# ruanyyyyyyy/point-cloud-process

Hardware: AMD Instinct MI355X
Metric: correspondence-pairs/sec + ms/ICP-iter, 120k-pt KITTI pair (higher is better)
Workload: dtype f64; 1 GPU; point-to-point ICP iteration, 120000 x 120000 KITTI-shaped synthetic scan pair per GPU (BASELINE configs[1]); exact 1-NN via grid; nn=grid, pairs_per_gpu=1, points_src=120000, points_tgt=120000

## Files before the change

point-cloud-process_amd/csrc/pcr_grid_search.hip:

```cpp
#include <atomic>
#include <chrono>
#include <cmath>
#include <cstdlib>
#include <cstring>
#include "pcr_grid_dev.h"
#include "pcr_icp_step.h"

#ifndef PCR_HARD_SCAN_T
#define PCR_HARD_SCAN_T 192
#endif
constexpr unsigned int HARD_SCAN_T = PCR_HARD_SCAN_T;
constexpr int HARD_STACK = 160;
constexpr long long ID_NONE = 0x7fffffffffffffffll;
constexpr int H_NLIST = 32;
constexpr int H_CSTRIDE = 32;
__host__ __device__ static inline unsigned int hard_list_cap(long long nq) {
    const long long tiles = (nq + 15) / 16;
    return (unsigned int)(((tiles + H_NLIST - 1) / H_NLIST) * 16 + 64);
}

template <int G>
__device__ static inline void group_best(double& bd2, long long& bid, unsigned int& bpos) {
#pragma unroll
    for (int off = G / 2; off > 0; off >>= 1) {
// ... 136 lines not shown
    unsigned long long dbg_pairs;
    unsigned int dbg_passes;
    unsigned long long probe;
};

struct wt_pre {
    pcr_pt p;
    unsigned int seed_pos;
    wt_xyz seed_b;
};
__device__ __forceinline__ static void wtile_preload(const unsigned int tile, const int lane, const pcr_pt* __restrict__ q, const long long nq,
                                                     const unsigned int* __restrict__ res_pos, const wt_xyz* __restrict__ prev_xyz, wt_pre& P) {
    const long long qi = (long long)tile * WT_Q + (lane & (WT_Q - 1));
    P.seed_pos = POS_NONE;
    P.seed_b = wt_xyz{0.0, 0.0, 0.0};
    P.p.x = P.p.y = P.p.z = 0.0; P.p.id = 0;
    if (qi < nq) {
        if (prev_xyz) {
            P.seed_pos = res_pos[qi];
            P.seed_b = prev_xyz[qi];
        }
        P.p = q[qi];
    }
}

#ifndef PCR_WT_WAVES
#define PCR_WT_WAVES 4
#endif
__device__ __forceinline__ static void wtile_search(const pcr_grid_view& gv, wtile_lds* L, const unsigned int tile, const int lane, const wt_pre& P,
                                                    pcr_pt* __restrict__ q, const long long nq, const pcr_xform& x, const int has_x, const int write_back,
                                                    const double max_d2, const int gated, const unsigned int pcap, unsigned int* __restrict__ res_pos,
                                                    double* __restrict__ res_d2, unsigned long long* __restrict__ dbg,
                                                    const wt_xyz* __restrict__ prev_xyz, wt_state& S, const unsigned long long* probe_p = nullptr,
                                                    const unsigned int probe_stride = 0, const unsigned int probe_groups = 0, const unsigned int probe_total = 0) {
#if !PCR_WT_MFMA
    typedef float f2 __attribute__((ext_vector_type(2)));
#endif
    typedef float f4 __attribute__((ext_vector_type(4)));
    const pcr_pt* __restrict__ g_pts = as_global(gv.pts);
#ifdef PCR_WT_DIAG
    const unsigned long long t_start = dbg ? __builtin_amdgcn_s_memtime() : 0;
    unsigned long long t_ph[8] = {0, 0, 0, 0, 0, 0, 0, 0}, t_last = t_start;
#define WT_STAMP(i) do { if (dbg) { const unsigned long long t_now = __builtin_amdgcn_s_memtime(); t_ph[i] += t_now - t_last; t_last = t_now; } } while (0)
#define WT_WHY(v) do { why = (v); } while (0)
    int why = 0;
#else
#define WT_STAMP(i) do {} while (0)
#define WT_WHY(v) do {} while (0)
#endif
    const long long qi = (long long)tile * WT_Q + (lane & (WT_Q - 1));
    const bool qvalid = qi < nq;
    double ax = 0, ay = 0, az = 0;
    bool clamped = false;
    const unsigned int seed_pos = P.seed_pos;
    const wt_xyz seed_b = P.seed_b;
    if (qvalid) {
        const pcr_pt p = P.p;
        ax = p.x; ay = p.y; az = p.z;
        if (has_x) {
            xform_apply(x, p, &ax, &ay, &az);
            if (write_back && lane < WT_Q) {
                pcr_pt o;
                o.x = ax; o.y = ay; o.z = az; o.id = p.id;
                q[qi] = o;
            }
        }
        cell_coord(ax, gv.lo[0], gv.inv_cell0, &clamped);
        cell_coord(ay, gv.lo[1], gv.inv_cell0, &clamped);
        cell_coord(az, gv.lo[2], gv.inv_cell0, &clamped);
    }
    
    WT_STAMP(0);
    bool open = qvalid;
    const float gate2 = gated ? (float)max_d2 * (1.0f + 1e-6f) : INFINITY;
    float bound2 = gate2;
    unsigned int cand_pos = POS_NONE, won = POS_NONE;
    if (prev_xyz && qvalid && !clamped) {
        const unsigned int pp = seed_pos;
        if (pp != POS_NONE) {
            const wt_xyz b = seed_b;
            const double dx = ax - b.x, dy = ay - b.y, dz = az - b.z;
            const float up = (float)((dx * dx + dy * dy) + dz * dz) * (1.0f + 2e-7f) + 1e-37f;
            if (up < bound2) { bound2 = up; cand_pos = pp; }
        }
    }
    unsigned long long dbg_pairs = 0, probe_v = 0;
    unsigned int dbg_passes = 0, staged = 0;
    const int max_passes = prev_xyz ? WT_PASSES_SEEDED : WT_PASSES;
    unsigned int staged_done = 0;
    float ring = 1.0f;
#pragma unroll 1
    for (int pass = 0; pass < max_passes; ++pass) {
        const bool part = open && !clamped;
        if (!__any(part)) break;
        if (pass > 0 && staged_done > (unsigned int)WT_HEAVY_STOP) break;
        int mn[3], mx[3];
        {
            const float rho = (cand_pos != POS_NONE) ? sqrtf(bound2) * (1.0f + 1e-6f) : fminf((float)gv.cell0 * ring, sqrtf(gate2));
            const double rc = fmin((double)rho * gv.inv_cell0, 262144.0);
            const double tx = (ax - gv.lo[0]) * gv.inv_cell0, ty = (ay - gv.lo[1]) * gv.inv_cell0, tz = (az - gv.lo[2]) * gv.inv_cell0;
            const int cmax = (int)PCR_COORD_MAX;
            mn[0] = part ? max(0, min(cmax, (int)floor(tx - rc) + (int)PCR_COORD_BIAS)) : 0x7fffffff;
            mx[0] = part ? max(0, min(cmax, (int)floor(tx + rc) + (int)PCR_COORD_BIAS)) : -1;
            mn[1] = part ? max(0, min(cmax, (int)floor(ty - rc) + (int)PCR_COORD_BIAS)) : 0x7fffffff;
            mx[1] = part ? max(0, min(cmax, (int)floor(ty + rc) + (int)PCR_COORD_BIAS)) : -1;
            mn[2] = part ? max(0, min(cmax, (int)floor(tz - rc) + (int)PCR_COORD_BIAS)) : 0x7fffffff;
            mx[2] = part ? max(0, min(cmax, (int)floor(tz + rc) + (int)PCR_COORD_BIAS)) : -1;
        }
#pragma unroll
        for (int k = 0; k < 3; ++k) {
            int lo_k = row16_min(mn[k]), hi_k = row16_max(mx[k]);
            if (WT_Q >= 32) {
                lo_k = min(__builtin_amdgcn_readlane(lo_k, 0), __builtin_amdgcn_readlane(lo_k, 16));
                hi_k = max(__builtin_amdgcn_readlane(hi_k, 0), __builtin_amdgcn_readlane(hi_k, 16));
            }
            if (WT_Q == 64) {
                const int lo2 = min(__builtin_amdgcn_readlane(row16_min(mn[k]), 32), __builtin_amdgcn_readlane(row16_min(mn[k]), 48));
// ... 286 lines not shown
#pragma unroll
        for (int off = WT_Q; off < 64; off <<= 1) {
            const float om = __shfl_xor(fm, off, 64), os = __shfl_xor(fs, off, 64);
            const unsigned int op = __shfl_xor(bpos, off, 64);
            fs = fminf(fmaxf(fm, om), fminf(fs, os));
            if (om < fm) { fm = om; bpos = op; }
        }
        if (part) {
            float U = INFINITY;
            bool ambiguous = false;
            if (bpos != POS_NONE) {
                const float R = 0.5f * cellLf * (float)max(d0, max(d1, d2));
                const float e = 8.0f * 5.9604644775390625e-08f * R * (1.0f + 1e-6f);
                const float dhi = sqrtf(fm) * (1.0f + 2e-6f) + e;
                U = (dhi + e) * (dhi + e) * (1.0f + 2e-6f);
                ambiguous = fs <= U;
            }
            float db = fminf(fminf(0.5f * d0 * cellLf - fabsf(qxf), 0.5f * d1 * cellLf - fabsf(qyf)), 0.5f * d2 * cellLf - fabsf(qzf));
            db = fmaxf(db - cellLf * (float)max(d0, max(d1, d2)) * 4e-6f, 0.0f);
            const float reach2 = fminf(U, bound2);
            if (!ambiguous && reach2 <= db * db * (1.0f - 2e-6f)) {
                open = false;
                won = bpos;
                if (lane < WT_Q) {
                    if (res_d2) {
                        double dd = DBL_MAX;
                        if (bpos != POS_NONE) {
                            const pcr_pt bb = g_pts[bpos];
                            dd = dist2(ax, ay, az, bb);
                        }
                        res_d2[qi] = dd;
                    }
                    if (!prev_xyz || bpos != seed_pos) res_pos[qi] = bpos;
                }
            } else {
                WT_WHY(ambiguous ? 3 : 4);
                if (bpos != POS_NONE && U < bound2) {
                    bound2 = U;
                    cand_pos = bpos;
                }
            }
        }
        ring = ring == 0.0f ? 1.0f : ring * 4.0f;
    }
    WT_STAMP(6);
    S.ax = ax; S.ay = ay; S.az = az;
    S.qi = qi;
    S.bound2 = bound2;
    S.cand_pos = cand_pos;
    S.won = won;
    S.open = open; S.clamped = clamped; S.qvalid = qvalid;
    S.staged = staged;
    S.dbg_pairs = dbg_pairs; S.dbg_passes = dbg_passes;
    {
        const bool ok = lane < (int)probe_groups && (unsigned int)probe_v == probe_total / (probe_groups ? probe_groups : 1u) + ((unsigned int)lane < probe_total % (probe_groups ? probe_groups : 1u) ? 1u : 0u);
        S.probe = (probe_groups && __ballot(ok) == (probe_groups >= 64 ? ~0ull : (1ull << probe_groups) - 1ull)) ? 1ull : 0ull;
    }
#ifdef PCR_WT_DIAG
    if (dbg) {
        const bool unres = open && lane < WT_Q;
        for (int r = 0; r < 5; ++r) {
            const unsigned int n_r = (unsigned int)__popcll(__ballot(unres && (clamped ? 0 : why) == r));
            if (lane == 0 && n_r) atomicAdd(&dbg[(1 << 15) + r], (unsigned long long)n_r);
        }
        if (lane == 0) {
            t_ph[7] = staged;
// ... 337 lines not shown
#ifndef PCR_ACC_SETS
#define PCR_ACC_SETS 32
#endif
constexpr int ACC_SETS = PCR_ACC_SETS;
#ifndef PCR_PASS_GROUPS
#define PCR_PASS_GROUPS 32
#endif
constexpr int PASS_GROUPS = PCR_PASS_GROUPS;
constexpr int PASS_SYNC_STRIDE = 32;
constexpr int PASS_SYNC_WORDS = PASS_SYNC_STRIDE * (PASS_GROUPS + 1);
constexpr unsigned long long ITEM_NONE = ~0ull;
constexpr unsigned int POISON_HI = 0xfffffffeu;
__device__ static inline unsigned long long item_poison(unsigned int pass_id) { return ((unsigned long long)POISON_HI << 32) | pass_id; }
#ifndef PCR_PASS_SPIN_LIMIT
#define PCR_PASS_SPIN_LIMIT (1u << 21)
#endif
constexpr unsigned int PASS_SPIN_LIMIT = PCR_PASS_SPIN_LIMIT;
constexpr int Q_BITS = 22;
constexpr unsigned long long Q_MASK = (1ull << Q_BITS) - 1ull;
constexpr long long PASS_MAX_NQ = 1ll << 26;
struct pass_args {
    unsigned long long* items;
    unsigned long long* sync;
    unsigned int cap;
    unsigned long long* acc;
    wt_xyz* prev_xyz;
    double scale, inv_scale;
    pcr_icp_dev_state* st;
    pcr_icp_loop_args la;
    unsigned int* tile_cost;
    unsigned int pass_id;
    unsigned long long* host_block;
    unsigned int notify;
    unsigned int* plog;
};
constexpr int PASS_LOG_WORDS = 3 * PCR_ICP_MAX_LOG + 8;
constexpr size_t HOST_LOG_OFF = (sizeof(pcr_icp_dev_state) + 63) & ~(size_t)63;
constexpr size_t HOST_FLAG_OFF = 8192 - 8;
static_assert(HOST_LOG_OFF + 4 * PASS_LOG_WORDS <= HOST_FLAG_OFF, "state + pass log + flag fit the landing block");
__host__ __device__ static inline unsigned int pass_item_cap(long long nq) {
    const long long tiles = (nq + WT_Q - 1) / WT_Q + 4;
    return (unsigned int)(((tiles + PASS_GROUPS - 1) / PASS_GROUPS) * (WT_Q + 1));
}

__device__ static inline long long to_fixed(double v, double scale) {
    constexpr double BIG = 6755399441055744.0;
    return __double_as_longlong(__builtin_fma(v, scale, BIG)) - __double_as_longlong(BIG);
}

__device__ static inline void acc_fixed_add(unsigned long long* __restrict__ acc, unsigned int set, int lane, double mk, double scale) {
    if (lane < PCR_NMOM - 1 && mk != 0.0)
        atomicAdd(acc + (size_t)(set % ACC_SETS) * PCR_NMOM + lane, (unsigned long long)to_fixed(mk, scale));
}

__device__ static inline void acc_fixed_add_ll(unsigned long long* __restrict__ acc, unsigned int set, int lane, long long v) {
    if (lane < PCR_NMOM - 1 && v != 0) atomicAdd(acc + (size_t)(set % ACC_SETS) * PCR_NMOM + lane, (unsigned long long)v);
}

__device__ static inline unsigned long long ld_dev(const unsigned long long* p) {
    return __hip_atomic_load(p, __ATOMIC_RELAXED, __HIP_MEMORY_SCOPE_AGENT);
}
__device__ static inline void st_dev(unsigned long long* p, unsigned long long v) {
    __hip_atomic_store(p, v, __ATOMIC_RELAXED, __HIP_MEMORY_SCOPE_AGENT);
}

union pass_lds {
    wtile_lds t;
    hard_lds h;
    double xch[WT_Q * (PCR_NMOM - 1)];
    long long xll[WT_Q * (PCR_NMOM - 1)];
};

__device__ __forceinline__ static void pass_serve_item(const pcr_grid_view& gv, pass_lds* L, const int lane, const unsigned long long w, const double max_d2,
                                                       const pass_args& A, unsigned int* __restrict__ res_pos, unsigned long long* __restrict__ dbg,
                                                       const unsigned int dbg_slot, const unsigned long long t_start) {
    const unsigned int w_lo = (unsigned int)w, w_hi = (unsigned int)(w >> 32);
    const double ax = __hiloint2double(__builtin_amdgcn_readlane((int)w_hi, 0), __builtin_amdgcn_readlane((int)w_lo, 0));
    const double ay = __hiloint2double(__builtin_amdgcn_readlane((int)w_hi, 1), __builtin_amdgcn_readlane((int)w_lo, 1));
    const double az = __hiloint2double(__builtin_amdgcn_readlane((int)w_hi, 2), __builtin_amdgcn_readlane((int)w_lo, 2));
    const unsigned int qi = (unsigned int)__builtin_amdgcn_readlane((int)w_lo, 3);
    const float cand_b2 = __uint_as_float((unsigned int)__builtin_amdgcn_readlane((int)w_hi, 3));
    const unsigned long long h_t0 = dbg ? __builtin_amdgcn_s_memtime() : 0;
    unsigned int h_steps = 0, h_pts = 0;
    int s_level0 = 0;
    double bd2;
    long long bid;
    unsigned int bpos;
    const bool have_cand = cand_b2 < INFINITY;
    double win[3];
    hard_search(gv, &L->h, lane, ax, ay, az, have_cand ? fmin((double)cand_b2, max_d2) : max_d2, have_cand, bd2, bid, bpos, h_steps, h_pts, s_level0, win);
    wave_sync();
    if (bpos != POS_NONE) {
        if (lane == 0) {
            pcr_pt b;
            b.x = win[0]; b.y = win[1]; b.z = win[2]; b.id = 0;
            A.prev_xyz[qi] = wt_xyz{b.x, b.y, b.z};
            double m[PCR_NMOM];
#pragma unroll
            for (int k = 0; k < PCR_NMOM; ++k) m[k] = 0.0;
            moments_add(m, gv.origin, ax, ay, az, b, max_d2, 1);
#pragma unroll
            for (int k = 0; k < PCR_NMOM - 1; ++k) L->xch[k] = m[k];
        }
        wave_sync();
        acc_fixed_add(A.acc, qi, lane, lane < PCR_NMOM - 1 ? L->xch[lane] : 0.0, A.scale);
        wave_sync();
    }
    if (lane == 0) {
        res_pos[qi] = bpos;
        if (dbg && dbg_slot < 60000) {
            dbg[(1 << 17) + dbg_slot * 4 + 0] = __builtin_amdgcn_s_memtime() - h_t0;
            dbg[(1 << 17) + dbg_slot * 4 + 1] = ((unsigned long long)h_steps << 32) | (unsigned int)((h_t0 - t_start) >> 4);
            dbg[(1 << 17) + dbg_slot * 4 + 2] = h_pts;
            dbg[(1 << 17) + dbg_slot * 4 + 3] = (unsigned long long)have_cand | ((unsigned long long)(s_level0 + 1) << 8);
        }
    }
}

__device__ __forceinline__ static void pass_finish(const pcr_grid_view& gv, pass_lds* L, const int lane, const pass_args& A, unsigned long long* root,
                                                   unsigned long long* __restrict__ dbg) {
    constexpr int HEAD_WORDS = (int)(pcr::ICP_STATE_HEAD_BYTES / 8);
    static_assert(pcr::ICP_STATE_HEAD_BYTES % 8 == 0 && HEAD_WORDS <= 64, "state head: one word per lane");
    double* const head = L->xch + 32;
    unsigned long long hw = 0, err_w = 0;
    if (lane < HEAD_WORDS) hw = reinterpret_cast<const unsigned long long*>(A.st)[lane];
    if (lane == 63) err_w = ld_dev(root + 16);
    const int mom = lane % PCR_NMOM, part = lane / PCR_NMOM;
    long long sum = 0;
    if (part < 3) {
        constexpr int PER = (ACC_SETS + 2) / 3;
        unsigned long long v[PER];
#pragma unroll
        for (int j = 0; j < PER; ++j) {
            const int set = part + 3 * j;
            v[j] = set < ACC_SETS ? ld_dev(A.acc + (size_t)set * PCR_NMOM + mom) : 0ull;
        }
#pragma unroll
        for (int j = 0; j < PER; ++j) {
            const int set = part + 3 * j;
            if (v[j]) st_dev(A.acc + (size_t)set * PCR_NMOM + mom, 0ull);
            sum += (long long)v[j];
        }
    }
    if (dbg && lane == 0) dbg[(1 << 19) - 4] = __builtin_amdgcn_s_memrealtime();
    sum += __shfl(sum, lane + PCR_NMOM, 64) + __shfl(sum, lane + 2 * PCR_NMOM, 64);
    wave_sync();
    if (dbg && lane == 0) dbg[(1 << 19) - 3] = __builtin_amdgcn_s_memrealtime();
// ... 130 lines not shown
                 pass_args A) {
    unsigned long long* const dbg = PCR_PASS_DIAG ? dbg_arg : nullptr;
    __shared__ pass_lds s_lds[4];
    const int lane = threadIdx.x & 63, wave = __builtin_amdgcn_readfirstlane((int)(threadIdx.x >> 6));
    const unsigned int tile = wtile_block(xcd_remap) * 4 + wave;
    wt_pre P;
    wtile_preload(tile, lane, q, nq, res_pos, use_prev ? A.prev_xyz : nullptr, P);
    const unsigned int last_cost = use_prev ? A.tile_cost[tile] : 0u;
    unsigned int pcap = pcap_arg;
    if (pcap_busy > pcap_arg && A.plog) {
        const unsigned int prev_items = A.pass_id > 0 && A.pass_id <= (unsigned int)PCR_ICP_MAX_LOG ? A.plog[2 * PCR_ICP_MAX_LOG + A.pass_id - 1] : 0xffffffffu;
        if ((unsigned long long)prev_items * 16ull > (unsigned long long)nq) pcap = pcap_busy;
        pcap = (unsigned int)__builtin_amdgcn_readfirstlane((int)pcap);
    }
    const pcr_xform x = A.st->x;
    if (A.st->stop) return;
    tile_set_priority(last_cost);
    const unsigned long long t_start = dbg ? __builtin_amdgcn_s_memtime() : 0;
    const unsigned long long rt_start = dbg ? __builtin_amdgcn_s_memrealtime() : 0;
    unsigned long long rt_tile = 0, rt_acc = 0;
    unsigned int n_items = 0, n_polls = 0, n_casfail = 0;
    pass_lds* L = &s_lds[wave];
    const unsigned int n_waves = gridDim.x * 4;
    const unsigned int g = tile % PASS_GROUPS;
    const unsigned int g_tiles = n_waves / PASS_GROUPS + (g < n_waves % PASS_GROUPS ? 1u : 0u);
    unsigned long long* const g_q = A.sync + (size_t)PASS_SYNC_STRIDE * g;
    unsigned long long* const g_started = g_q + 16;
    unsigned long long* const g_ticket = g_q + 17;
    unsigned long long* const items = A.items + (size_t)g * A.cap * 4;
    if (lane == 0) __hip_atomic_fetch_add(g_started, 1ull, __ATOMIC_RELAXED, __HIP_MEMORY_SCOPE_AGENT);
    const unsigned int n_groups = n_waves < (unsigned int)PASS_GROUPS ? n_waves : (unsigned int)PASS_GROUPS;
    wt_state S;
    wtile_search(*gvp, &L->t, tile, lane, P, q, nq, x, 1, 1, max_d2, 1, pcap, res_pos, nullptr, dbg, use_prev ? A.prev_xyz : nullptr, S, inline_queue ? A.sync + 16 : nullptr,
                 (unsigned int)PASS_SYNC_STRIDE, n_groups, n_waves);
    tile_record_cost(S, lane, A.tile_cost, tile);
    if (dbg) rt_tile = __builtin_amdgcn_s_memrealtime();
    tile_nb nb;
    tile_neighbour(gv.pts, S, P, lane, nb);
    bool all_started = false;
    if (inline_queue) {
        all_started = S.probe != 0;
        if (!all_started) {
            unsigned long long sv = 0;
            if (lane < (int)n_groups) sv = ld_dev(A.sync + (size_t)PASS_SYNC_STRIDE * lane + 16);
            const bool ok = lane < (int)n_groups && (unsigned int)sv == n_waves / PASS_GROUPS + ((unsigned int)lane < n_waves % PASS_GROUPS ? 1u : 0u);
            all_started = __ballot(ok) == (n_groups >= 64 ? ~0ull : (1ull << n_groups) - 1ull);
        }
    }
    const bool unres = S.open && lane < WT_Q;
    const unsigned long long um = __ballot(unres);
    unsigned int mine = 0;
    bool have_claim = false;
    unsigned long long own = 0;
    unsigned long long* const root = A.sync + (size_t)PASS_SYNC_STRIDE * PASS_GROUPS;
    {
        unsigned int tg;
        const unsigned long long slot_w = publish_reserve(A.sync, um, unres, lane, g, n_groups, tg);
        asm volatile("" :: "v"(slot_w) : "memory");
        if (lane == 0)
            own = __hip_atomic_fetch_add(g_q, (1ull << (2 * Q_BITS)) | (all_started ? 1ull << Q_BITS : 0ull), __ATOMIC_RELAXED, __HIP_MEMORY_SCOPE_AGENT);
        if (unres) publish_store<true>(A.items, A.cap, tg, slot_w, S, (unsigned int)S.qi);
    }
    tile_fold_moments(L, lane, S, P, nb, gv.origin, max_d2, A.prev_xyz, A.scale, A.acc, tile);
    wave_sync();
    {
        {
            const unsigned int o_lo = (unsigned int)__builtin_amdgcn_readfirstlane((int)(unsigned int)own), o_hi = (unsigned int)__builtin_amdgcn_readfirstlane((int)(unsigned int)(own >> 32));
// ... 49 lines not shown
                const unsigned int q_lo = (unsigned int)__builtin_amdgcn_readfirstlane((int)(unsigned int)qw), q_hi = (unsigned int)__builtin_amdgcn_readfirstlane((int)(unsigned int)(qw >> 32));
                qw = ((unsigned long long)q_hi << 32) | q_lo;
                mine = (unsigned int)((qw >> Q_BITS) & Q_MASK);
                if (mine >= (unsigned int)(qw & Q_MASK)) break;
                int got = 0;
                if (lane == 0) {
                    unsigned long long expect = qw;
                    got = __hip_atomic_compare_exchange_strong(g_q, &expect, qw + (1ull << Q_BITS), __ATOMIC_RELAXED, __ATOMIC_RELAXED, __HIP_MEMORY_SCOPE_AGENT) ? 1 : 0;
                }
                if (!__builtin_amdgcn_readfirstlane(got)) { ++n_casfail; continue; }
            }
        }
        have_claim = false;
        unsigned long long* it = items + (size_t)mine * 4;
        unsigned long long w = ITEM_NONE;
        bool poisoned = false;
        for (unsigned int spins = 0;; ++spins) {
            if (lane < 4) w = ld_dev(it + lane);
            const unsigned int w3_lo = (unsigned int)__builtin_amdgcn_readlane((int)(unsigned int)w, 3), w3_hi = (unsigned int)__builtin_amdgcn_readlane((int)(unsigned int)(w >> 32), 3);
            poisoned = w3_hi == POISON_HI && w3_lo == A.pass_id;
            const unsigned long long mk = __ballot(lane < 4 && w != ITEM_NONE && !(lane == 3 && w3_hi == POISON_HI));
            if (poisoned || mk == 0xfull) break;
            if (spins >= PASS_SPIN_LIMIT) { failed = true; break; }
            ++n_polls;
#ifndef PCR_SLOT_SLEEP
#define PCR_SLOT_SLEEP 16
#endif
            __builtin_amdgcn_s_sleep(PCR_SLOT_SLEEP);
        }
        if (failed) break;
        if (poisoned) { left_by_poison = true; break; }
        if (lane < 4) st_dev(it + lane, ITEM_NONE);
        ++n_items;
        pass_serve_item(gv, L, lane, w, max_d2, A, res_pos, dbg, g + PASS_GROUPS * mine, t_start);
    }
    const unsigned long long rt_loop = dbg ? __builtin_amdgcn_s_memrealtime() : 0;
    asm volatile("s_waitcnt vmcnt(0)" ::: "memory");
    int last = 0;
    {
        if (lane == 0) {
            const unsigned long long tg_old = __hip_atomic_fetch_add(g_ticket, 1ull | (left_by_poison ? 1ull << 32 : 0ull) | (failed ? 1ull << 48 : 0ull), __ATOMIC_RELAXED,
                                                                     __HIP_MEMORY_SCOPE_AGENT);
            if ((unsigned int)tg_old == g_tiles - 1u) {
                const bool g_clean = ((tg_old >> 32) & 0xffffull) != 0 || left_by_poison;
                const bool g_failed = (tg_old >> 48) != 0 || failed;
                const unsigned long long tr_old = __hip_atomic_fetch_add(root, 1ull | (g_clean ? 1ull << 32 : 0ull) | (g_failed ? 1ull << 48 : 0ull), __ATOMIC_RELAXED,
                                                                         __HIP_MEMORY_SCOPE_AGENT);
                if ((unsigned int)tr_old == n_groups - 1u) {
                    last = ((unsigned int)((tr_old >> 32) & 0xffffull) + (g_clean ? 1u : 0u) == n_groups) ? 1 : 2;
                    if ((tr_old >> 48) != 0 || g_failed) last = 3;
                }
            }
        }
    }
    if (dbg && lane == 0) {
        unsigned long long* d = dbg + (1 << 19) + (size_t)(blockIdx.x * 4 + wave) * 8;
        d[0] = rt_start; d[1] = rt_tile; d[2] = rt_acc; d[3] = rt_loop; d[4] = n_items; d[5] = n_polls | ((unsigned long long)n_casfail << 32); d[6] = S.dbg_pairs | ((unsigned long long)S.dbg_passes << 40) | ((unsigned long long)__popcll(um) << 48); d[7] = __builtin_amdgcn_s_memrealtime();
    }
    last = __builtin_amdgcn_readfirstlane(last);
    if (!last) return;
    if (last == 3 && dbg_arg && lane == 0) atomicAdd(&dbg_arg[(1 << 19) - 16], 1ull);
    if (last >= 2) {
        unsigned long long qw = 0;
        if (lane < (int)n_groups) qw = ld_dev(A.sync + (size_t)PASS_SYNC_STRIDE * lane);
        const unsigned int r_l = (unsigned int)(qw & Q_MASK);
        const unsigned int c_l = last == 3 ? 0u : (unsigned int)((qw >> Q_BITS) & Q_MASK);
        unsigned long long left = __ballot(lane < (int)n_groups && c_l < r_l);
        while (left) {
            const int gg = (int)__ffsll((long long)left) - 1;
            left &= left - 1;
            const unsigned int c0 = (unsigned int)__builtin_amdgcn_readlane((int)c_l, gg), r0 = (unsigned int)__builtin_amdgcn_readlane((int)r_l, gg);
            for (unsigned int i = c0; i < r0; ++i) {
                unsigned long long* it = A.items + ((size_t)gg * A.cap + i) * 4;
                unsigned long long w = ITEM_NONE;
                bool arrived = false;
                const unsigned int patience = last == 3 ? 64u : (PASS_SPIN_LIMIT < (1u << 21) ? (1u << 21) : PASS_SPIN_LIMIT);
                bool served_before = false;
                for (unsigned int spins = 0; spins < patience; ++spins) {
                    if (lane < 4) w = ld_dev(it + lane);
                    const unsigned int w3_hi = (unsigned int)__builtin_amdgcn_readlane((int)(unsigned int)(w >> 32), 3);
                    if (__ballot(lane < 4 && w != ITEM_NONE && !(lane == 3 && w3_hi == POISON_HI)) == 0xfull) { arrived = true; break; }
                    if (last == 3 && __ballot(lane < 4 && w == ITEM_NONE) == 0xfull) { served_before = true; break; }
                    __builtin_amdgcn_s_sleep(2);
                }
                if (served_before) continue;
                if (lane < 4) st_dev(it + lane, ITEM_NONE);
                if (!arrived) { if (lane == 0) st_dev(root + 16, 1ull); continue; }
                pass_serve_item(gv, L, lane, w, max_d2, A, res_pos, dbg, 59999u, t_start);
            }
        }
        asm volatile("s_waitcnt vmcnt(0)" ::: "memory");
    }
    if (lane < (int)n_groups) {
        st_dev(A.sync + (size_t)PASS_SYNC_STRIDE * lane, 0ull);
        st_dev(A.sync + (size_t)PASS_SYNC_STRIDE * lane + 16, 0ull);
        st_dev(A.sync + (size_t)PASS_SYNC_STRIDE * lane + 17, 0ull);
    }
    if (lane == 0) st_dev(root, 0ull);
    pass_finish(gv, L, lane, A, root, dbg);
}

__global__ void __launch_bounds__(256) __attribute__((amdgpu_waves_per_eu(PCR_WT_WAVES, 8)))
grid_drain_kernel(pcr_grid_view gv, double max_d2, unsigned int* __restrict__ res_pos, unsigned long long* __restrict__ dbg, pass_args A) {
    __shared__ pass_lds s_lds[4];
    if (A.st->stop) return;
    const unsigned long long t_start = dbg ? __builtin_amdgcn_s_memtime() : 0;
    const unsigned long long t_rt_start = __builtin_amdgcn_s_memrealtime();
    const int lane = threadIdx.x & 63, wave = threadIdx.x >> 6;
    pass_lds* L = &s_lds[wave];
    const drain_part dp = drain_partition(A.sync, lane);
    const unsigned int total = dp.total;
    const unsigned int n_waves = gridDim.x * 4;
    if (dbg && blockIdx.x == 0 && threadIdx.x == 0) dbg[(1 << 19) - 8] = total;
    if (A.plog && blockIdx.x == 0 && threadIdx.x == 0 && A.pass_id < (unsigned int)PCR_ICP_MAX_LOG) {
        A.plog[PCR_ICP_MAX_LOG + A.pass_id] = (unsigned int)t_rt_start | 1u;
        A.plog[2 * PCR_ICP_MAX_LOG + A.pass_id] = total;
    }
    for (unsigned int w_i = blockIdx.x * 4 + wave; w_i < total; w_i += n_waves)
        pass_serve_item(gv, L, lane, drain_take(dp, A.items, A.cap, w_i, lane), max_d2, A, res_pos, dbg, w_i, t_start);
    asm volatile("s_waitcnt vmcnt(0)" ::: "memory");
    unsigned long long* const root = A.sync + (size_t)PASS_SYNC_STRIDE * PASS_GROUPS;
    const unsigned int wid = blockIdx.x * 4 + wave;
    const unsigned int n_groups = n_waves < (unsigned int)PASS_GROUPS ? n_waves : (unsigned int)PASS_GROUPS;
    const unsigned int g = wid % n_groups;
    const unsigned int g_size = n_waves / n_groups + (g < n_waves % n_groups ? 1u : 0u);
    unsigned long long* const g_ticket = A.sync + (size_t)PASS_SYNC_STRIDE * g + 17;
    int last = 0;
    if (lane == 0) {
        if (__hip_atomic_fetch_add(g_ticket, 1ull, __ATOMIC_RELAXED, __HIP_MEMORY_SCOPE_AGENT) == (unsigned long long)(g_size - 1u)) {
            st_dev(g_ticket, 0ull);
            if (__hip_atomic_fetch_add(root, 1ull, __ATOMIC_RELAXED, __HIP_MEMORY_SCOPE_AGENT) == (unsigned long long)(n_groups - 1u)) {
                st_dev(root, 0ull);
                last = 1;
            }
        }
    }
    if (!__builtin_amdgcn_readfirstlane(last)) return;
    if (lane < PASS_GROUPS) {
        st_dev(A.sync + (size_t)PASS_SYNC_STRIDE * lane, 0ull);
        st_dev(A.sync + (size_t)PASS_SYNC_STRIDE * lane + 16, 0ull);
    }
    pass_finish(gv, L, lane, A, root, dbg);
}

__global__ void grid_finalize_nn1_kernel(pcr_grid_view gv, const pcr_pt* __restrict__ q, long long nq, const unsigned int* __restrict__ res_pos,
                                         const double* __restrict__ res_d2, double max_d2, int gated, int* __restrict__ idx_out,
                                         double* __restrict__ d2_out, unsigned int* __restrict__ hard_count) {
    const long long qi = (long long)blockIdx.x * blockDim.x + threadIdx.x;
    if (qi < H_NLIST) hard_count[H_CSTRIDE * qi] = 0;
    if (qi >= nq) return;
    const unsigned int pos = res_pos[qi];
    const double d2 = res_d2[qi];
// ... 272 lines not shown
    const loop_guard in_flight(ctx->device);
    const auto h_t0 = std::chrono::steady_clock::now();
    auto h_us = [&](std::chrono::steady_clock::time_point a) { return std::chrono::duration_cast<std::chrono::nanoseconds>(std::chrono::steady_clock::now() - a).count() / 1e3; };
    for (double& v : ctx->pass_host_us) v = 0.0;
    const char* const wait_s = getenv("PCR_PASS_INLINE");
    const int wait_env = wait_s ? atoi(wait_s) : -1;
    const bool gated = (params->max_d2 > 0) && std::isfinite(params->max_d2);
    int rc = pcr_cloud_morton_sort(ctx, qc, idx->cell);
    if (rc) return rc;
    const int64_t nq = qc->n;
    int grid = (int)((nq + 1023) / 1024);
    if (grid > ctx->cu_count) grid = ctx->cu_count;
    double sc_f = 0, sc_i = 0;
    const bool fused = gated && nq <= PASS_MAX_NQ && getenv("PCR_ICP_NO_FUSED") == nullptr &&
                       pcr_pass_fixed_scale(idx->lo, idx->hi, nq, params->max_d2, &sc_f, &sc_i);
    grid_scratch sc(ctx);
    pcr_dev_block st_blk(ctx);
    if ((rc = grid_scratch_alloc(&sc, nq, false, !fused)) || (rc = sc.prev_xyz.alloc(24 * (size_t)nq))) return rc;
    const pass_layout pl = pass_scratch_layout(nq, 1, true);
    pass_args pa{};
    if (fused) {
        if ((rc = sc.acc.alloc(8 * pl.zero_words)) || (rc = sc.tile_cost.alloc(sizeof(unsigned int) * 4 * (size_t)wtile_blocks(nq))) ||
            (rc = sc.items.alloc(8 * pl.item_words)))
            return rc;
        pa.cap = pl.cap;
        pa.items = sc.items.as<unsigned long long>();
        pa.tile_cost = sc.tile_cost.as<unsigned int>();
        pa.acc = sc.acc.as<unsigned long long>();
        pa.sync = pa.acc + pl.sync_word;
        pa.plog = (unsigned int*)(pa.acc + pl.log_word);
        pa.prev_xyz = sc.prev_xyz.as<wt_xyz>();
        pa.scale = sc_f;
        pa.inv_scale = sc_i;
    }
    if ((rc = pcr_ensure_scratch(ctx, sizeof(double) * PCR_NMOM * (size_t)grid)) || (rc = st_blk.alloc(sizeof(pcr_icp_dev_state)))) return rc;
    pcr_icp_dev_state* const d_st = st_blk.as<pcr_icp_dev_state>();
    static_assert(sizeof(pcr_icp_dev_state) <= 8192, "state must fit the pinned staging buffer");
    pcr_icp_dev_state* h_st = (pcr_icp_dev_state*)ctx->h_state;
    memset(h_st, 0, sizeof(*h_st));
    pcr::icp_state_from_T0(T0, h_st);
    const pcr_icp_loop_args la = pcr_icp_loop_args_from(params);
    volatile unsigned long long* const h_flag = (volatile unsigned long long*)((char*)ctx->h_state + HOST_FLAG_OFF);
    if (fused) {
        void* dp = nullptr;
        if (hipHostGetDevicePointer(&dp, ctx->h_state, 0) == hipSuccess) pa.host_block = (unsigned long long*)dp;
        *h_flag = 0ull;
        h_flag[-1] = 0ull;
    }
    hipError_t e = hipSuccess;
    ctx->pass_host_us[0] = h_us(h_t0);
    if (fused) {
        pass_T0 t0;
        for (int i = 0; i < 16; ++i) t0.v[i] = T0[i];
        const int ib = (int)((pl.item_words + 256 * 8 - 1) / (256 * 8));
        hipLaunchKernelGGL(pass_init_kernel, dim3(ib < 1 ? 1 : (ib > 1024 ? 1024 : ib)), dim3(256), 0, ctx->stream, pa.acc, (unsigned int)pl.zero_words,
                           pa.items, pl.item_words, d_st, t0, pa.plog,
                           pa.host_block ? pa.host_block + HOST_FLAG_OFF / 8 - 1 : (unsigned long long*)nullptr);
        e = hipGetLastError();
    } else e = hipMemcpyAsync(d_st, h_st, sizeof(*h_st), hipMemcpyHostToDevice, ctx->stream);
    pa.st = d_st;
    pa.la = la;
    pcr_xform xi;
    pcr_xform_from_T(nullptr, &xi);
    int enq = 0;
    const double prof_before = ctx->prof_ms[0] + ctx->prof_ms[1] + ctx->prof_ms[2] + ctx->prof_ms[3];
    int chunk = params->min_iter > 2 ? params->min_iter : 2;
    if (ctx->profile) chunk = 1;
    while (e == hipSuccess && rc == PCR_OK && enq < params->max_iter) {
        if (chunk > params->max_iter - enq) chunk = params->max_iter - enq;
        if (chunk > 64) chunk = 64;
        for (int c = 0; c < chunk && rc == PCR_OK; ++c) {
            const bool use_prev = enq + c > 0;
            const bool one_generation = (nq + WT_Q - 1) / WT_Q <= 16ll * ctx->cu_count;
            const int inline_queue = wait_env >= 0 ? wait_env : ((one_generation && !ctx->shared_device && in_flight.n.load(std::memory_order_relaxed) == 1) ? 1 : 0);
            if (fused) {
                if (ctx->profile) pcr_prof_mark(ctx, 0);
                if (ctx->d_debug) hipMemsetAsync(ctx->d_debug, 0, sizeof(unsigned long long) * (inline_queue ? ((1 << 16) + 8 * (size_t)((nq + 63) / 64)) : ((size_t)1 << 19)), ctx->stream);
                pa.pass_id = (unsigned int)(enq + c);
                pa.notify = c == chunk - 1 ? 1u : 0u;
                const unsigned int cap_n = wtile_point_cap(ctx, nq), cap_busy = (!inline_queue && cap_n > (unsigned int)(WT_PR * WT_ROUNDS_SMALL)) ? WT_BUSY_CAP : cap_n;
                hipLaunchKernelGGL(grid_pass_kernel, dim3(wtile_blocks(nq)), dim3(256), 0, ctx->stream, (const pcr_grid_view*)idx->d_view, idx->view, qc->d, (long long)nq,
                                   params->max_d2, WT_XCD_REMAP, cap_n, cap_busy, sc.res_pos.as<unsigned int>(), ctx->d_debug, use_prev ? 1 : 0, inline_queue, pa);
                if (ctx->profile) pcr_prof_mark(ctx, 1);
                if (!inline_queue)
                    hipLaunchKernelGGL(grid_drain_kernel, dim3(queue_blocks(ctx, (nq + 3) / 4)), dim3(256), 0, ctx->stream, idx->view, params->max_d2,
                                       sc.res_pos.as<unsigned int>(), ctx->d_debug, pa);
                if (hipGetLastError() != hipSuccess) { rc = PCR_E_HIP; break; }
                pcr_prof_mark(ctx, 2);
            } else {
                rc = grid_search_enqueue(ctx, idx, qc->d, nq, ctx->stream, nullptr, 1, params->max_d2, gated, ctx->profile, &sc, d_st, use_prev);
                if (rc) break;
                pcr_prof_mark(ctx, 2);
                hipLaunchKernelGGL(grid_accumulate_kernel, dim3(grid), dim3(256), 0, ctx->stream, idx->view, (const pcr_pt*)qc->d, (long long)nq, xi,
                                   0, (const unsigned int*)sc.res_pos.p, params->max_d2, gated ? 1 : 0, ctx->d_partials, ctx->d_counters + 64,
                                   (double*)nullptr, sc.hard_count, d_st, la, sc.prev_xyz.as<wt_xyz>());
            }
            pcr_prof_mark(ctx, 3);
            pcr_prof_mark(ctx, 4);
            pcr_prof_finish(ctx);
        }
        enq += chunk;
        if (rc) break;
        if (ctx->pass_host_us[1] == 0.0) ctx->pass_host_us[1] = h_us(h_t0) - ctx->pass_host_us[0];
        const auto h_tw = std::chrono::steady_clock::now();
        if (pa.host_block) {
            bool seen = false;
            for (unsigned int spins = 0;; ++spins) {
                if (ctx->pass_host_us[4] == 0.0 && h_flag[-1] != 0ull) ctx->pass_host_us[4] = h_us(h_t0);
                const unsigned long long f = __atomic_load_n((const unsigned long long*)h_flag, __ATOMIC_ACQUIRE);
                if (f >= (unsigned long long)enq || (f > 0 && h_st->stop)) { seen = true; break; }
                if ((spins & 255u) == 255u && h_us(h_tw) > 2e6) break;
                __builtin_ia32_pause();
            }
            ctx->pass_host_us[5] = h_us(h_tw);
            if (!seen) {
                e = pcr_sync(ctx->stream);
                if (e == hipSuccess && pcr_d2h_small(ctx, h_st, d_st, sizeof(*h_st)) != PCR_OK) e = hipErrorUnknown;
            }
        } else {
            hipEventRecord(ctx->ev3, ctx->stream);
            if (pcr_d2h_small_enqueue(ctx, h_st, d_st, sizeof(*h_st)) != PCR_OK) e = hipErrorUnknown;
            if (e == hipSuccess && fused && pcr_d2h_small_enqueue(ctx, (char*)ctx->h_state + HOST_LOG_OFF, pa.plog, 4 * PASS_LOG_WORDS) != PCR_OK) e = hipErrorUnknown;
            double flag_us = 0.0;
            if (e == hipSuccess && pcr_wait_flag(ctx, &flag_us) != PCR_OK) e = hipErrorUnknown;
            ctx->pass_host_us[5] = flag_us;
            { float ms = 0; if (hipEventElapsedTime(&ms, ctx->ev0, ctx->ev3) == hipSuccess) ctx->pass_host_us[4] = 1e3 * ms; }
        }
        ctx->pass_host_us[2] += h_us(h_tw);
        if (e != hipSuccess || h_st->stop) break;
        if (!ctx->profile) chunk *= 2;
    }
    if (e == hipSuccess) e = hipGetLastError();
    ctx->pass_log_n = 0;
    ctx->loop_dev_ms = 0.0;
    if (e == hipSuccess && rc == PCR_OK && fused) {
        const unsigned int* const lg = (const unsigned int*)((const char*)ctx->h_state + HOST_LOG_OFF);
        const int np = h_st->passes < PCR_ICP_MAX_LOG ? h_st->passes : PCR_ICP_MAX_LOG;
        unsigned int prev = lg[3 * PCR_ICP_MAX_LOG];
        for (int k = 0; k < np; ++k) {
            const unsigned int end = lg[k], ds = lg[PCR_ICP_MAX_LOG + k];
            ctx->pass_log[0][k] = 0.01 * (double)(unsigned int)((ds ? ds : end) - prev);
            ctx->pass_log[1][k] = ds ? 0.01 * (double)(unsigned int)(end - ds) : 0.0;
            ctx->pass_log[2][k] = (double)lg[2 * PCR_ICP_MAX_LOG + k];
// ... 42 lines not shown
    const unsigned int n_groups = n_waves < (unsigned int)PASS_GROUPS ? n_waves : (unsigned int)PASS_GROUPS;
    const double max_d2 = B.max_d2;
    wt_state S;
    wtile_search(bp->gv, &L->t, tile, lane, P, q, nq, x, 1, 1, max_d2, 1, pcap, res_pos, nullptr, nullptr, use_prev ? prev_xyz : nullptr, S);
    tile_record_cost(S, lane, B.tile_cost, tile_g);
    tile_nb nb;
    tile_neighbour(bp->gv.pts, S, P, lane, nb);
    const bool unres = S.open && lane < WT_Q;
    const unsigned long long um = __ballot(unres);
    if (um) {
        unsigned int tg;
        const unsigned long long slot_w = publish_reserve(B.sync, um, unres, lane, g, n_groups, tg);
        if (unres) publish_store<false>(B.items, B.cap, tg, slot_w, S, (unsigned int)(q_off + (unsigned long long)S.qi));
    }
    tile_fold_moments(L, lane, S, P, nb, bp->gv.origin, max_d2, prev_xyz, bp->scale, B.acc + (size_t)p * ACC_SETS * PCR_NMOM, tile);
}

__global__ void __launch_bounds__(256) __attribute__((amdgpu_waves_per_eu(PCR_WT_WAVES, 8)))
batch_drain_kernel(pcr_batch_pass_args B) {
    __shared__ pass_lds s_lds[4];
    const int lane = threadIdx.x & 63, wave = threadIdx.x >> 6;
    pass_lds* L = &s_lds[wave];
    const drain_part dp = drain_partition(B.sync, lane);
    const unsigned int n_waves = gridDim.x * 4;
    for (unsigned int w_i = blockIdx.x * 4 + wave; w_i < dp.total; w_i += n_waves) {
        const unsigned long long w = drain_take(dp, B.items, B.cap, w_i, lane);
        const unsigned int slot = (unsigned int)__builtin_amdgcn_readlane((int)(unsigned int)w, 3);
        const unsigned int p = (unsigned int)__builtin_amdgcn_readfirstlane((int)as_global(B.tile_pair)[slot / WT_Q]);
        const pcr_batch_pair* const bp = batch_pair_ptr(B, p);
        pass_args A{};
        A.acc = B.acc + (size_t)p * ACC_SETS * PCR_NMOM;
        A.prev_xyz = (wt_xyz*)B.prev_xyz;
        A.scale = bp->scale;
        pass_serve_item(bp->gv, L, lane, w, B.max_d2, A, B.res_pos, nullptr, w_i, 0ull);
    }
}

__global__ void __launch_bounds__(256)
batch_finish_kernel(pcr_batch_pass_args B, unsigned int pass_id) {
    __shared__ pass_lds s_lds[4];
    const int lane = threadIdx.x & 63, wave = threadIdx.x >> 6;
    if (blockIdx.x == 0 && wave == 0 && lane < PASS_GROUPS) B.sync[(size_t)PASS_SYNC_STRIDE * lane] = 0ull;
    const unsigned int p = (unsigned int)__builtin_amdgcn_readfirstlane((int)(blockIdx.x * 4 + wave));
    if (p >= (unsigned int)B.n_pairs) return;
    pcr_icp_dev_state* const st = B.st + p;
    if (as_global(st)->stop) return;
    const pcr_batch_pair* const bp = batch_pair_ptr(B, p);
    if (bp->nq <= 0) return;
    pass_lds* L = &s_lds[wave];
    pass_args A{};
    A.acc = B.acc + (size_t)p * ACC_SETS * PCR_NMOM;
    A.st = st;
    A.la = B.la;
    A.inv_scale = bp->inv_scale;
    unsigned long long* const root = B.sync + (size_t)PASS_SYNC_STRIDE * PASS_GROUPS;
    pass_finish(bp->gv, L, lane, A, root, nullptr);
    wave_sync();
    if (lane == 0 && !reinterpret_cast<const pcr_icp_dev_state*>(L->xch + 32)->stop) atomicAdd(B.running + pass_id, 1u);
}

__global__ void __launch_bounds__(256)
batch_init_kernel(unsigned long long* __restrict__ zero_p, unsigned long long zero_n, unsigned long long* __restrict__ ones_p, unsigned long long ones_n,
                  unsigned int* __restrict__ running, pcr_icp_dev_state* __restrict__ st, int n_pairs, const double* __restrict__ T0) {
    pass_fill(ones_p, ones_n, zero_p, zero_n);
    for (unsigned long long i = (unsigned long long)blockIdx.x * blockDim.x + threadIdx.x; i < PCR_ICP_MAX_LOG + 1; i += (unsigned long long)gridDim.x * blockDim.x)
        running[i] = 0u;
    for (int p = blockIdx.x; p < n_pairs; p += gridDim.x) {
// ... 39 lines not shown
```

Baseline: 3.378 billion correspondences/s.

## Cache far-query bounds to skip hard searches for points beyond max distance

Adds a far-point bound: when a query with no seed candidate finds no neighbor within a slightly enlarged probe radius (1.25x the max distance), the hard search stores the query position in prev_xyz as a marker. On the next ICP iteration, a query with no seed that has moved less than the guaranteed margin is closed immediately without searching. The intent is to avoid repeatedly paying for expensive hard searches on outlier points that cannot match, at the cost of a wider probe radius on first search and extra state writes. It also fixes the host flag wait to compare the stop flag against the current chunk and zeros the pass log.

```diff
diff --git a/point-cloud-process_amd/csrc/pcr_grid_search.hip b/point-cloud-process_amd/csrc/pcr_grid_search.hip
--- a/point-cloud-process_amd/csrc/pcr_grid_search.hip
+++ b/point-cloud-process_amd/csrc/pcr_grid_search.hip
@@ -192,7 +192,8 @@
                                                     const double max_d2, const int gated, const unsigned int pcap, unsigned int* __restrict__ res_pos,
                                                     double* __restrict__ res_d2, unsigned long long* __restrict__ dbg,
                                                     const wt_xyz* __restrict__ prev_xyz, wt_state& S, const unsigned long long* probe_p = nullptr,
-                                                    const unsigned int probe_stride = 0, const unsigned int probe_groups = 0, const unsigned int probe_total = 0) {
+                                                    const unsigned int probe_stride = 0, const unsigned int probe_groups = 0, const unsigned int probe_total = 0,
+                                                    wt_xyz* far_xyz = nullptr, const double far_m2 = 0.0) {
 #if !PCR_WT_MFMA
     typedef float f2 __attribute__((ext_vector_type(2)));
 #endif
@@ -243,6 +244,10 @@
             const float up = (float)((dx * dx + dy * dy) + dz * dz) * (1.0f + 2e-7f) + 1e-37f;
             if (up < bound2) { bound2 = up; cand_pos = pp; }
         }
+    }
+    if (far_xyz && prev_xyz && qvalid && seed_pos == POS_NONE) {
+        const double dx = ax - seed_b.x, dy = ay - seed_b.y, dz = az - seed_b.z;
+        if ((dx * dx + dy * dy) + dz * dz < far_m2) open = false;
     }
     unsigned long long dbg_pairs = 0, probe_v = 0;
     unsigned int dbg_passes = 0, staged = 0;
@@ -595,6 +600,7 @@
                         res_d2[qi] = dd;
                     }
                     if (!prev_xyz || bpos != seed_pos) res_pos[qi] = bpos;
+                    if (far_xyz && bpos == POS_NONE && (!prev_xyz || seed_pos != POS_NONE)) far_xyz[qi].x = __longlong_as_double(0x7ff8000000000000ll);
                 }
             } else {
                 WT_WHY(ambiguous ? 3 : 4);
@@ -998,6 +1004,7 @@
     unsigned int pass_id;
     unsigned long long* host_block;
     unsigned int notify;
+    double far_p2, far_m2;
     unsigned int* plog;
 };
 constexpr int PASS_LOG_WORDS = 3 * PCR_ICP_MAX_LOG + 8;
@@ -1037,6 +1044,22 @@
     long long xll[WT_Q * (PCR_NMOM - 1)];
 };
 
+#ifndef PCR_FAR_BOUND
+#define PCR_FAR_BOUND 1
+#endif
+#ifndef PCR_FAR_PROBE
+#define PCR_FAR_PROBE 1.25
+#endif
+static void pass_far_bounds(double max_d2, double* far_p2, double* far_m2) {
+    const double e = ldexp(1.0, -40);
+    const double p2 = max_d2 * (PCR_FAR_PROBE * PCR_FAR_PROBE);
+    const double lim = (sqrt(p2) * (1.0 - e) - sqrt(max_d2) * (1.0 + e)) / (1.0 + e);
+    const bool on = PCR_FAR_BOUND && std::isfinite(p2) && lim > 0.0 && getenv("PCR_FAR_BOUND_OFF") == nullptr;
+    *far_p2 = on ? p2 : max_d2;
+    *far_m2 = on ? lim * lim * (1.0 - e) : 0.0;
+}
+
+template <bool FAR>
 __device__ __forceinline__ static void pass_serve_item(const pcr_grid_view& gv, pass_lds* L, const int lane, const unsigned long long w, const double max_d2,
                                                        const pass_args& A, unsigned int* __restrict__ res_pos, unsigned long long* __restrict__ dbg,
                                                        const unsigned int dbg_slot, const unsigned long long t_start) {
@@ -1054,8 +1077,14 @@
     unsigned int bpos;
     const bool have_cand = cand_b2 < INFINITY;
     double win[3];
-    hard_search(gv, &L->h, lane, ax, ay, az, have_cand ? fmin((double)cand_b2, max_d2) : max_d2, have_cand, bd2, bid, bpos, h_steps, h_pts, s_level0, win);
+    const bool probe = FAR && !have_cand && A.far_m2 > 0.0;
+    hard_search(gv, &L->h, lane, ax, ay, az, have_cand ? fmin((double)cand_b2, max_d2) : (probe ? A.far_p2 : max_d2), have_cand, bd2, bid, bpos, h_steps, h_pts, s_level0, win);
     wave_sync();
+    const bool far = probe && !(bd2 < A.far_p2);
+    if (far) {
+        if (lane == 0) A.prev_xyz[qi] = wt_xyz{ax, ay, az};
+        bpos = POS_NONE;
+    }
     if (bpos != POS_NONE) {
         if (lane == 0) {
             pcr_pt b;
@@ -1078,7 +1107,7 @@
             dbg[(1 << 17) + dbg_slot * 4 + 0] = __builtin_amdgcn_s_memtime() - h_t0;
             dbg[(1 << 17) + dbg_slot * 4 + 1] = ((unsigned long long)h_steps << 32) | (unsigned int)((h_t0 - t_start) >> 4);
             dbg[(1 << 17) + dbg_slot * 4 + 2] = h_pts;
-            dbg[(1 << 17) + dbg_slot * 4 + 3] = (unsigned long long)have_cand | ((unsigned long long)(s_level0 + 1) << 8);
+            dbg[(1 << 17) + dbg_slot * 4 + 3] = (unsigned long long)have_cand | (!(bd2 < max_d2) ? 2ull : 0ull) | (far ? 4ull : 0ull) | ((unsigned long long)(s_level0 + 1) << 8);
         }
     }
 }
@@ -1275,7 +1304,7 @@
     const unsigned int n_groups = n_waves < (unsigned int)PASS_GROUPS ? n_waves : (unsigned int)PASS_GROUPS;
     wt_state S;
     wtile_search(*gvp, &L->t, tile, lane, P, q, nq, x, 1, 1, max_d2, 1, pcap, res_pos, nullptr, dbg, use_prev ? A.prev_xyz : nullptr, S, inline_queue ? A.sync + 16 : nullptr,
-                 (unsigned int)PASS_SYNC_STRIDE, n_groups, n_waves);
+                 (unsigned int)PASS_SYNC_STRIDE, n_groups, n_waves, A.far_m2 > 0.0 ? A.prev_xyz : nullptr, A.far_m2);
     tile_record_cost(S, lane, A.tile_cost, tile);
     if (dbg) rt_tile = __builtin_amdgcn_s_memrealtime();
     tile_nb nb;
@@ -1391,7 +1420,7 @@
         if (poisoned) { left_by_poison = true; break; }
         if (lane < 4) st_dev(it + lane, ITEM_NONE);
         ++n_items;
-        pass_serve_item(gv, L, lane, w, max_d2, A, res_pos, dbg, g + PASS_GROUPS * mine, t_start);
+        pass_serve_item<true>(gv, L, lane, w, max_d2, A, res_pos, dbg, g + PASS_GROUPS * mine, t_start);
     }
     const unsigned long long rt_loop = dbg ? __builtin_amdgcn_s_memrealtime() : 0;
     asm volatile("s_waitcnt vmcnt(0)" ::: "memory");
@@ -1445,7 +1474,7 @@
                 if (served_before) continue;
                 if (lane < 4) st_dev(it + lane, ITEM_NONE);
                 if (!arrived) { if (lane == 0) st_dev(root + 16, 1ull); continue; }
-                pass_serve_item(gv, L, lane, w, max_d2, A, res_pos, dbg, 59999u, t_start);
+                pass_serve_item<true>(gv, L, lane, w, max_d2, A, res_pos, dbg, 59999u, t_start);
             }
         }
         asm volatile("s_waitcnt vmcnt(0)" ::: "memory");
@@ -1476,7 +1505,7 @@
         A.plog[2 * PCR_ICP_MAX_LOG + A.pass_id] = total;
     }
     for (unsigned int w_i = blockIdx.x * 4 + wave; w_i < total; w_i += n_waves)
-        pass_serve_item(gv, L, lane, drain_take(dp, A.items, A.cap, w_i, lane), max_d2, A, res_pos, dbg, w_i, t_start);
+        pass_serve_item<true>(gv, L, lane, drain_take(dp, A.items, A.cap, w_i, lane), max_d2, A, res_pos, dbg, w_i, t_start);
     asm volatile("s_waitcnt vmcnt(0)" ::: "memory");
     unsigned long long* const root = A.sync + (size_t)PASS_SYNC_STRIDE * PASS_GROUPS;
     const unsigned int wid = blockIdx.x * 4 + wave;
@@ -1815,12 +1844,14 @@
         pa.prev_xyz = sc.prev_xyz.as<wt_xyz>();
         pa.scale = sc_f;
         pa.inv_scale = sc_i;
+        pass_far_bounds(params->max_d2, &pa.far_p2, &pa.far_m2);
     }
     if ((rc = pcr_ensure_scratch(ctx, sizeof(double) * PCR_NMOM * (size_t)grid)) || (rc = st_blk.alloc(sizeof(pcr_icp_dev_state)))) return rc;
     pcr_icp_dev_state* const d_st = st_blk.as<pcr_icp_dev_state>();
     static_assert(sizeof(pcr_icp_dev_state) <= 8192, "state must fit the pinned staging buffer");
     pcr_icp_dev_state* h_st = (pcr_icp_dev_state*)ctx->h_state;
     memset(h_st, 0, sizeof(*h_st));
+    memset((char*)ctx->h_state + HOST_LOG_OFF, 0, 4 * PASS_LOG_WORDS);
     pcr::icp_state_from_T0(T0, h_st);
     const pcr_icp_loop_args la = pcr_icp_loop_args_from(params);
     volatile unsigned long long* const h_flag = (volatile unsigned long long*)((char*)ctx->h_state + HOST_FLAG_OFF);
@@ -1852,6 +1883,7 @@
     while (e == hipSuccess && rc == PCR_OK && enq < params->max_iter) {
         if (chunk > params->max_iter - enq) chunk = params->max_iter - enq;
         if (chunk > 64) chunk = 64;
+        const unsigned long long enq_before = (unsigned long long)enq;
         for (int c = 0; c < chunk && rc == PCR_OK; ++c) {
             const bool use_prev = enq + c > 0;
             const bool one_generation = (nq + WT_Q - 1) / WT_Q <= 16ll * ctx->cu_count;
@@ -1891,7 +1923,7 @@
             for (unsigned int spins = 0;; ++spins) {
                 if (ctx->pass_host_us[4] == 0.0 && h_flag[-1] != 0ull) ctx->pass_host_us[4] = h_us(h_t0);
                 const unsigned long long f = __atomic_load_n((const unsigned long long*)h_flag, __ATOMIC_ACQUIRE);
-                if (f >= (unsigned long long)enq || (f > 0 && h_st->stop)) { seen = true; break; }
+                if (f >= (unsigned long long)enq || (f > enq_before && h_st->stop)) { seen = true; break; }
                 if ((spins & 255u) == 255u && h_us(h_tw) > 2e6) break;
                 __builtin_ia32_pause();
             }
@@ -2000,7 +2032,7 @@
         A.acc = B.acc + (size_t)p * ACC_SETS * PCR_NMOM;
         A.prev_xyz = (wt_xyz*)B.prev_xyz;
         A.scale = bp->scale;
-        pass_serve_item(bp->gv, L, lane, w, B.max_d2, A, B.res_pos, nullptr, w_i, 0ull);
+        pass_serve_item<false>(bp->gv, L, lane, w, B.max_d2, A, B.res_pos, nullptr, w_i, 0ull);
     }
 }
 
```

Result: no change. 3.394 billion correspondences/s (median of 6 runs) (+0.5%).
